# matsengrp/linearham

Measured on AMD Instinct MI355X. Metric: phylo-HMM log-likelihood evals/sec (100-leaf x 400-site family), higher is better.
Workload: dtype f64

## Files before the change

### linearham_amd/csrc/lh_capi.hip

```cpp
#include <algorithm>
#include <array>
#include <map>
#include <cstdio>
#include <cstring>
#include <functional>
#include <atomic>
#include <chrono>
#include <string>
#include <thread>
#include <utility>
#include <vector>

#include "lh_device.h"

namespace lh {
const DebugOptions& debug_options() {
  static const DebugOptions opts = [] {
    DebugOptions o;
    auto set = [](const char* name) { return std::getenv(name) != nullptr; };
    auto num = [](const char* name, int dflt) { const char* e = std::getenv(name); return e ? std::atoi(e) : dflt; };
    o.chunk = std::max(256, num("LH_CHUNK", o.chunk));
    o.host_sub = std::max(256, num("LH_HOST_SUB", o.host_sub));
    o.eval_split = std::min(8, std::max(0, num("LH_EVAL_SPLIT", o.eval_split)));
    o.eval_fwd_priority = std::min(1, num("LH_EVAL_FWD_PRIORITY", o.eval_fwd_priority));
    o.k2b_no_pair = set("LH_K2B_NO_PAIR");
    o.k2b_vd_single = set("LH_K2B_VD_SINGLE");
    o.sample_timing = set("LH_SAMPLE_TIMING");
    o.k1_tile_cap = num("LH_K1_TILE_CAP", 0);
    o.k1_cxx_walk = set("LH_K1_CXX_WALK");
    o.k1_tables = set("LH_K1_TABLES");
    o.k1_stack = set("LH_K1_STACK");
    o.k1_no_tables = set("LH_K1_NO_TABLES");
    o.k1_segments = set("LH_K1_SEGMENTS");
    o.k1_seg_waves = num("LH_K1_SEG_WAVES", o.k1_seg_waves);
    o.k1_no_fuse = set("LH_K1_NO_FUSE");
    o.codon_blocks = std::max(1, num("LH_CODON_BLOCKS", o.codon_blocks));
    o.events_blocks = std::max(1, num("LH_EVENTS_BLOCKS", o.events_blocks));
    o.anc_out_mb = std::max(1, num("LH_ANC_OUT_MB", o.anc_out_mb));
    o.edge_out_mb = std::max(1, num("LH_EDGE_OUT_MB", o.edge_out_mb));
    o.collect_hash_bits = std::min(64, std::max(1, num("LH_COLLECT_HASH_BITS", o.collect_hash_bits)));
    return o;
  }();
  return opts;
}
}

namespace {

thread_local std::string g_error;

int fail(const std::string& msg) {
  g_error = msg;
  return 1;
}

#define LH_HIP(expr)                                                                      \
  do {                                                                                    \
    hipError_t e_ = (expr);                                                               \
    if (e_ != hipSuccess)                                                                 \
      return fail(std::string(#expr) + ": " + hipGetErrorString(e_));                     \
  } while (0)

template <bool Pinned>
class Buffer {
 public:
  Buffer() = default;
  Buffer(const Buffer&) = delete;
  Buffer& operator=(const Buffer&) = delete;
  ~Buffer() { release(); }
  int ensure(size_t bytes) {
    bytes = std::max<size_t>(bytes, 64);
    if (bytes <= cap_) return 0;
    if (p_) {
      LH_HIP(hipDeviceSynchronize());
      release();
    }
// ... 199 lines not shown
struct SeqStore {
  DevBuf ids, flag, pairs;
  DevBuf gather_slots, gather_out;
  DevBuf store[2];
  int cur = 0;
  int32_t K = 0;
  size_t cap = 0;
};

struct CollectWs {
  DevBuf seqs, hash, states;
  int32_t n_last = -1;
  SeqStore store;
};

struct LineageWs {
  DevBuf naive, path, nt_hash, aa_hash;
  lh::LineageBatch last{};
  SeqStore store;
  LineageWs() { last.n = -1; }
};

struct HostInputs {
  DevBuf ops, brlen, er, pi, alpha;
  DevBuf rates, naive;
  DevBuf words;
  DevBuf log_offset;
  DevBuf em;
};
struct HostOutputs {
  DevBuf loglik, rates, xmsa_emission, forward, scaler_counts;
  DevBuf states;
  DevBuf anc, rate_choice;
  DevBuf weighted_sum, weight_stats;
  DevBuf log_cand, log_prior;
  DevBuf log_path;
};

struct HostPipe {
  PinnedBuf pinned[2];
  hipStream_t copy = nullptr, comp = nullptr;
  hipEvent_t staged[2] = {nullptr, nullptr};
  ~HostPipe() {
    for (hipEvent_t e : staged)
      if (e) (void)hipEventDestroy(e);
    if (copy) (void)hipStreamDestroy(copy);
    if (comp) (void)hipStreamDestroy(comp);
  }
};

struct OverlapPipe {
  static constexpr int kMaxSplit = 8;
  hipStream_t prune = nullptr, fwd = nullptr;
  hipEvent_t fork = nullptr, join_prune = nullptr, join_fwd = nullptr;
  hipEvent_t pruned[kMaxSplit] = {};
  bool ready = false;
  int ensure(bool fwd_high) {
    if (ready) return 0;
    int least = 0, greatest = 0;
    LH_HIP(hipDeviceGetStreamPriorityRange(&least, &greatest));
    if (!prune) LH_HIP(hipStreamCreateWithFlags(&prune, hipStreamNonBlocking));
    if (!fwd) LH_HIP(hipStreamCreateWithPriority(&fwd, hipStreamNonBlocking, fwd_high ? greatest : 0));
    for (hipEvent_t* e : {&fork, &join_prune, &join_fwd})
      if (!*e) LH_HIP(hipEventCreateWithFlags(e, hipEventDisableTiming));
    for (hipEvent_t& e : pruned)
      if (!e) LH_HIP(hipEventCreateWithFlags(&e, hipEventDisableTiming));
    ready = true;
    return 0;
  }
  ~OverlapPipe() {
    for (hipEvent_t e : {fork, join_prune, join_fwd})
      if (e) (void)hipEventDestroy(e);
    for (hipEvent_t e : pruned)
      if (e) (void)hipEventDestroy(e);
    if (prune) (void)hipStreamDestroy(prune);
    if (fwd) (void)hipStreamDestroy(fwd);
  }
};

}

struct lh_family {
  int device = 0;
  lh::DevFamily host{};
  lh::DevFamily* dev = nullptr;
  std::vector<void*> allocs;
  char* arena_ptr = nullptr;
  size_t arena_left = 0;
  Workspace ws;
  ForwardWs fws;
  AsrWs asr;
  PosteriorWs post;
  CandidateWs cand;
  ViterbiWs vit;
  CodonSource codon_src;
  CodonWs codon;
  EventsWs events;
  CollectWs collect;
  LineageWs lineage;
  AncestralWs anc;
  EdgesWs edges;
  DevBuf forward_dev;
  HostInputs in;
  HostOutputs out;
  PinnedBuf staging;
  HostPipe pipe;
  OverlapPipe overlap;
  bool profile = false;
  KernelTimer<3> eval_timer;
  KernelTimer<1> asr_timer, post_timer;
  KernelTimer<1> prior_timer, cand_timer;
  KernelTimer<1> collect_timer;
  KernelTimer<1> vit_timer;
  KernelTimer<1> codon_timer;
  KernelTimer<2> events_timer;
  KernelTimer<1> lineage_timer;
  KernelTimer<3> anc_timer;
  KernelTimer<3> edges_timer;
  KernelTimer<5> chain_timer;
  bool extended = false;
  bool have_sampler = false;
  lh::DevSampler sampler{};
  const lh::DevSampler* sampler_dev = nullptr;
  int32_t n_ucol_used = 0;
// ... 303 lines not shown

struct TreeBatch {
  int32_t n, T, max_depth;
  const int32_t* ops;
  const double* brlen;
  const double* er;
  const double* pi;
  const double* model;
  int32_t R;
  bool per_rate = false;
  size_t nodes() const { return 2 * (size_t)T - 2; }
  size_t n_ops() const { return (size_t)T - 2; }
  size_t model_stride() const { return per_rate ? (size_t)R : 1; }
  bool has_arrays() const { return ops && brlen && er && pi && model; }
  const int32_t* schedule(size_t i) const { return ops + i * n_ops() * 4; }
  TreeBatch slice(size_t off, int32_t m) const {
    return {m, T, max_depth, schedule(off), brlen + off * nodes(), er + off * 6, pi + off * 4, model + off * model_stride(),
            R, per_rate};
  }
  std::array<size_t, 5> sample_bytes() const {
    return {sizeof(int32_t) * 4 * n_ops(), sizeof(double) * nodes(), sizeof(double) * 6, sizeof(double) * 4,
            sizeof(double) * model_stride()};
  }
};

int check_batch(const lh_family* f, const std::string& w, const TreeBatch& b, bool needs_sampler = false) {
  const int n = b.n, T = b.T, R = b.R, max_depth = b.max_depth;
  if (!f) return fail(w + ": null family");
  if (needs_sampler && !f->have_sampler) return fail(w + ": lh_family_set_sampler has not been called");
  if (n < 0) return fail(w + ": negative batch size");
  if (n == 0) return -1;
  if (f->host.n_seqs < 1) return fail(w + ": family was created without an MSA (forward-only)");
  if (T != f->host.n_seqs + 1) return fail(w + ": n_tips must equal n_seqs + 1 (naive)");
  if (T < 3) return fail(w + ": need at least 3 tips");
  if (R < 1 || R > 64) return fail(w + ": num_rates out of range");
  if (max_depth < 0 || max_depth > 16) return fail(w + ": max_depth out of range");
  if ((size_t)T * 128 > 160 * 1024) return fail(w + ": too many tips for the LDS tip table");
  return 0;
}

size_t eval_bytes_per_sample(const lh_family* f, int T, int R) {
  return k1_bytes_per_sample(f, T, R) + sizeof(double) * R * 6 * (size_t)std::max(f->host.n_prune, 1);
}

size_t eval_group(const lh_family* f, int T, int R) {
  return std::min<size_t>(kChunk, std::max<size_t>(1024, ((size_t)16 << 30) / eval_bytes_per_sample(f, T, R)));
}

size_t asr_group(const lh_family* f, int T, int R, size_t clv_per_sample) {
  return std::min<size_t>(8192, std::max<size_t>(64, ((size_t)8 << 30) / (clv_per_sample + eval_bytes_per_sample(f, T, R))));
}

int prune_group(lh_family* f, const std::string& who, const TreeBatch& g, const double* rates, bool mix, hipStream_t stream,
                int* planes, size_t row0 = 0, int row0_planes = 0) {
  Workspace& w = f->ws;
  const lh::PruneWsSizes z = lh::prune_ws_sizes(g.T, f->host.msa_mixed_n != 0);
  const size_t L = (size_t)std::max(f->host.n_prune, 0), pl = (size_t)row0_planes;
  lh::PruneWs p = w.prune;
  p.scratch += row0 * g.R * z.scratch_doubles_per_rate;
  p.wops += row0 * g.n_ops();
  p.wlen += row0 * g.n_ops();
  p.tabs += row0 * z.tabs_per_sample;
  p.hdr += row0;
  *planes = lh::launch_prune(f->host, g.n, g.R, g.T, g.max_depth, g.ops, g.brlen, rates, w.eig.get<double>() + row0 * 36, p, g.pi,
                             w.site_lik.get<double>() + row0 * pl * 5 * L, w.site_scal.get<int32_t>() + row0 * pl * L, stream,
                             mix, f->extended || !mix);
  if (*planes < 0) return fail(who + ": " + lh::prune_last_error());
  f->k1_form = lh::prune_last_form();
  if (!mix && *planes != g.R && f->host.n_prune > 0) return fail(who + ": internal error (rate planes were mixed)");
  if (row0 > 0 && *planes != row0_planes) return fail(who + ": internal error (sub-batches with different rate planes)");
  return 0;
}

bool valid_op(const int32_t* op, int T, int nodes, int max_depth) {
  const int kind = op[0] & 15;
  const bool push = op[0] & lh::OP_PUSH_FLAG;
  const int rank = op[0] >> lh::OP_RANK_SHIFT;
  bool ok = (op[0] & 0xe0) == 0 && op[0] >= 0 && kind <= 2 && rank <= T - 3;
  if (kind == lh::OP_CHERRY) ok = ok && op[1] >= 1 && op[1] < T && op[2] >= 1 && op[2] < T;
  if (kind == lh::OP_TIP_ACC) ok = ok && !push && op[1] >= 1 && op[1] < T && op[2] >= T && op[2] < nodes;
  if (kind == lh::OP_POP_ACC) ok = ok && !push && op[1] >= T && op[1] < nodes && op[2] >= T && op[2] < nodes;
  if (push || kind == lh::OP_POP_ACC) ok = ok && op[3] >= 0 && op[3] < max_depth;
  return ok;
}

bool valid_schedule(const int32_t* ops, int T, int nodes, int max_depth) {
  int count = 0, depth = 0;
  for (int k = 0; k < T - 2; ++k) {
    const int32_t* op = ops + (size_t)k * 4;
    if (!valid_op(op, T, nodes, max_depth)) return false;
    const int kind = op[0] & 15, rank = op[0] >> lh::OP_RANK_SHIFT;
    if (kind == lh::OP_CHERRY) {
      if (rank != 0 && rank != count) return false;
      if (((op[0] & lh::OP_PUSH_FLAG) != 0) != (k != 0)) return false;
      if (k != 0 && op[3] != depth++) return false;
    } else {
      if (rank != count) return false;
      count += kind == lh::OP_POP_ACC ? 2 : 1;
      if (kind == lh::OP_POP_ACC && op[3] != --depth) return false;
    }
  }
  return count == T - 3 && depth == 0;
}

template <typename Fn>
void in_threads(size_t n, int nw, Fn&& fn) {
  if (nw <= 1) return fn((size_t)0, n);
  std::vector<std::thread> pool;
  for (int t = 0; t < nw; ++t) pool.emplace_back(fn, n * t / nw, n * (t + 1) / nw);
  for (std::thread& th : pool) th.join();
}

bool valid_schedules(const TreeBatch& b) {
  const size_t n = b.n;
  const int nw = (int)std::max<size_t>(1, std::min<size_t>({(size_t)std::thread::hardware_concurrency(), (size_t)8, n * b.n_ops() / 65536}));
  std::atomic<bool> bad{false};
  in_threads(n, nw, [&](size_t lo, size_t hi) {
    for (size_t i = lo; i < hi && !bad; ++i)
      if (!valid_schedule(b.schedule(i), b.T, (int)b.nodes(), b.max_depth)) bad = true;
// ... 618 lines not shown
      return fail("lh_family_set_sampler: D-J junction dimensions differ from the family's");
    if (upload_sampler_junction(f, desc->dj, &s.dj)) return 1;
    draws += (s.n_d >= 2) + s.dj.n_rows;
    s.states_per_sample += 1 + s.dj.n_rows;
  }
  s.words_per_sample = 2 * draws;
  f->sampler = s;
  if (upload(f, &s, 1, &f->sampler_dev)) return 1;
  f->have_sampler = true;
  return 0;
}

int32_t lh_sample_words(const lh_family* f) { return f && f->have_sampler ? f->sampler.words_per_sample : 0; }
int32_t lh_sample_states(const lh_family* f) { return f && f->have_sampler ? f->sampler.states_per_sample : 0; }

int lh_family_status(lh_family* f) {
  if (!f) return fail("lh_family_status: null family");
  DeviceGuard guard(f);
  return check_async_error(f, "lh_family_status");
}

int lh_profile_enable(lh_family* f, int enable) {
  if (!f) return fail("null family");
  f->profile = enable != 0;
  return 0;
}

int lh_profile_read(lh_family* f, double* ms_model, double* ms_prune, double* ms_forward, int64_t* n_launches) {
  double ms[3];
  if (profile_read(f, &lh_family::eval_timer, ms, n_launches)) return 1;
  if (ms_model) *ms_model = ms[0];
  if (ms_prune) *ms_prune = ms[1];
  if (ms_forward) *ms_forward = ms[2];
  return 0;
}

int lh_asr_profile_read(lh_family* f, double* ms_sampling, int64_t* n_launches) {
  return profile_read(f, &lh_family::asr_timer, ms_sampling, n_launches);
}

namespace {

constexpr int kEvalSplit = 1;
constexpr bool kEvalFwdHigh = false;
static_assert(kEvalSplit >= 1 && kEvalSplit <= OverlapPipe::kMaxSplit, "one `pruned` event per sub-batch");
int eval_sub_batch(int m) {
  const int forced = lh::debug_options().eval_split;
  if (forced > 0) return (m + forced - 1) / forced;
  constexpr int kBlock = 6144;
  if (kEvalSplit <= 1 || m < 2 * kBlock) return m;
  return ((m + kEvalSplit - 1) / kEvalSplit + kBlock - 1) / kBlock * kBlock;
}

int eval_group_split(lh_family* f, const TreeBatch& g, int off, int per, double* rates, double* em_out, double* loglik,
                     const lh_eval_outputs* outs, const lh::LogEmRequest& lem, hipStream_t stream) {
  OverlapPipe& op = f->overlap;
  const int fwd_priority = lh::debug_options().eval_fwd_priority;
  if (op.ensure(fwd_priority < 0 ? kEvalFwdHigh : fwd_priority > 0)) return 1;
  Workspace& w = f->ws;
  const int m = g.n, R = g.R;
  const size_t C = f->host.n_xmsa, L = (size_t)std::max(f->host.n_prune, 0);
  KernelTimer<3>* timer = f->profile ? &f->eval_timer : nullptr;
  LH_HIP(hipEventRecord(op.fork, stream));
  LH_HIP(hipStreamWaitEvent(op.prune, op.fork, 0));
  LH_HIP(hipStreamWaitEvent(op.fwd, op.fork, 0));
  auto enqueue = [&]() -> int {
    if (timer) timer->begin_spans();
    if (timer && timer->span_begin(0, op.prune)) return 1;
    lh::launch_model_setup(m, R, g.er, g.pi, g.model, rates, w.eig.get<double>(), op.prune);
    if (timer && timer->span_end(op.prune)) return 1;
    int planes = 0;
    for (int r0 = 0, j = 0; r0 < m; r0 += per, ++j) {
      const int k = std::min(per, m - r0);
      const TreeBatch sub = g.slice(r0, k);
      if (timer && timer->span_begin(1, op.prune)) return 1;
      if (prune_group(f, "lh_eval_batch", sub, rates + (size_t)r0 * R, true, op.prune, &planes, r0, planes)) return 1;
      if (timer && timer->span_end(op.prune)) return 1;
      LH_HIP(hipEventRecord(op.pruned[j], op.prune));
      LH_HIP(hipStreamWaitEvent(op.fwd, op.pruned[j], 0));
      if (timer && timer->span_begin(2, op.fwd)) return 1;
      const size_t s0 = (size_t)off + r0;
      const lh::LogEmRequest lem_k{lem.cols, lem.n, lem.out ? lem.out + s0 * lem.n : nullptr};
      if (run_forward(f, k, planes, w.site_lik.get<double>() + (size_t)r0 * planes * 5 * L,
                      w.site_scal.get<int32_t>() + (size_t)r0 * planes * L, sub.pi, nullptr,
                      em_out ? em_out + (size_t)r0 * C : nullptr, loglik + s0, outs, s0, op.fwd, lem_k, r0, m))
        return 1;
      if (timer && timer->span_end(op.fwd)) return 1;
    }
    if (timer) timer->end_spans();
    return 0;
  };
  const int rc = enqueue();
  LH_HIP(hipEventRecord(op.join_prune, op.prune));
  LH_HIP(hipEventRecord(op.join_fwd, op.fwd));
  LH_HIP(hipStreamWaitEvent(stream, op.join_prune, 0));
  LH_HIP(hipStreamWaitEvent(stream, op.join_fwd, 0));
  return rc;
}

int eval_device(lh_family* f, const TreeBatch& b, double* loglik, const lh_eval_outputs* outs, void* hip_stream,
                const lh::LogEmRequest& lem = lh::LogEmRequest{}, const std::function<int(int, int)>* after = nullptr) {
  if (int rc = check_batch(f, "lh_eval_batch", b)) return rc > 0;
  DeviceGuard guard(f);
  if (!b.has_arrays() || !loglik) return fail("lh_eval_batch: null array");
  hipStream_t stream = static_cast<hipStream_t>(hip_stream);
  const int n = b.n, R = b.R;
  const int chunk = (int)std::min<size_t>(n, eval_group(f, b.T, R));
  if (ensure_workspace(f, chunk, R, b.T)) return 1;
  Workspace& w = f->ws;
  double *eig = w.eig.get<double>(), *site_lik = w.site_lik.get<double>();
  int32_t* site_scal = w.site_scal.get<int32_t>();
  const size_t C = f->host.n_xmsa;
  for (int off = 0; off < n; off += chunk) {
    const int m = std::min(chunk, n - off);
    const TreeBatch g = b.slice(off, m);
    double* rates = (outs && outs->rates) ? outs->rates + (size_t)off * R : w.rates.get<double>();
    double* em_out = (outs && outs->xmsa_emission) ? outs->xmsa_emission + (size_t)off * C : nullptr;
    if (const int per = eval_sub_batch(m); per < m) {
      if (eval_group_split(f, g, off, per, rates, em_out, loglik, outs, lem, stream)) return 1;
      LH_HIP(hipGetLastError());
      if (after && (*after)(off, m)) return 1;
      continue;
    }
    if (f->profile && f->eval_timer.begin(stream)) return 1;
    lh::launch_model_setup(m, R, g.er, g.pi, g.model, rates, eig, stream);
    if (f->profile && f->eval_timer.mark(1, stream)) return 1;
    int planes = 0;
    if (prune_group(f, "lh_eval_batch", g, rates, true, stream, &planes)) return 1;
    if (f->profile && f->eval_timer.mark(2, stream)) return 1;
    const lh::LogEmRequest lem_m{lem.cols, lem.n, lem.out ? lem.out + (size_t)off * lem.n : nullptr};
    if (run_forward(f, m, planes, site_lik, site_scal, g.pi, nullptr, em_out, loglik + off, outs, off, stream, lem_m))
      return 1;
    if (f->profile && f->eval_timer.end(stream)) return 1;
    LH_HIP(hipGetLastError());
    if (after && (*after)(off, m)) return 1;
  }
  return 0;
}

}

int lh_eval_batch_device(lh_family* f, int32_t n, int32_t T, int32_t max_depth, const int32_t* ops,
                         const double* brlen, const double* er, const double* pi, const double* alpha,
                         int32_t R, double* loglik, const lh_eval_outputs* outs, void* hip_stream) {
  return eval_device(f, {n, T, max_depth, ops, brlen, er, pi, alpha, R}, loglik, outs, hip_stream);
}

int lh_eval_batch(lh_family* f, int32_t n, int32_t T, int32_t max_depth, const int32_t* ops,
                  const double* brlen, const double* er, const double* pi, const double* alpha, int32_t R,
                  double* loglik, const lh_eval_outputs* outs) {
  const TreeBatch host{n, T, max_depth, ops, brlen, er, pi, alpha, R};
  if (int rc = check_batch(f, "lh_eval_batch", host)) return rc > 0;
  DeviceGuard guard(f);
  if (!host.has_arrays() || !loglik) return fail("lh_eval_batch: null array");
  const size_t C = f->host.n_xmsa, FS = f->host.forward_size, SS = f->host.scaler_size;
  const lh_eval_outputs none{};
  const lh_eval_outputs& o = outs ? *outs : none;
  HostOutputs& out = f->out;
  lh_eval_outputs d_outs{};
  if (out.loglik.ensure(sizeof(double) * n) || out_buf(o.rates, out.rates, sizeof(double) * R * n, &d_outs.rates) ||
      out_buf(o.xmsa_emission, out.xmsa_emission, sizeof(double) * C * n, &d_outs.xmsa_emission) ||
      out_buf(o.forward, out.forward, sizeof(double) * FS * n, &d_outs.forward) ||
      out_buf(o.scaler_counts, out.scaler_counts, sizeof(int32_t) * SS * n, &d_outs.scaler_counts))
    return 1;
  double* d_ll = out.loglik.get<double>();

  const std::array<size_t, 5> bytes = host.sample_bytes();
  const char* src[5] = {(const char*)ops, (const char*)brlen, (const char*)er, (const char*)pi, (const char*)alpha};
  DevBuf* in[5] = {&f->in.ops, &f->in.brlen, &f->in.er, &f->in.pi, &f->in.alpha};
  char* dst[5];
  size_t per_sample = 0;
  for (int a = 0; a < 5; ++a) {
    if (in[a]->ensure(bytes[a] * n)) return 1;
    dst[a] = in[a]->get<char>();
    per_sample += bytes[a];
  }
  const TreeBatch dev{n, T, max_depth, (const int32_t*)dst[0], (const double*)dst[1], (const double*)dst[2],
                      (const double*)dst[3], (const double*)dst[4], R};
  const int kSub = lh::debug_options().host_sub;
  const int sub = std::min<int>(n, kSub);
  HostPipe& hp = f->pipe;
// ... 2059 lines not shown
```

### linearham_amd/csrc/lh_device.h

```cpp
#pragma once
#include <hip/hip_runtime.h>
#include <stdint.h>

#include "linearham_amd.h"

namespace lh {

constexpr double kScaleFactor = 0x1p256;
constexpr double kScaleThreshold = 0x1p-256;
constexpr double kLogScaleFactor = 177.445678223345993274;

enum : int { OP_CHERRY = 0, OP_TIP_ACC = 1, OP_POP_ACC = 2, OP_PUSH_FLAG = 16, OP_RANK_SHIFT = 8 };

enum : int { W_CHERRY = 0, W_TIP_ACC = 1, W_POP = 2, W_CTIP = 3, W_CTAB_ACC = 4 };

struct PruneWs {
  double* scratch;
  int2* wops;
  double* wlen;
  int4* tabs;
  int4* hdr;
  int32_t* err_flag;
};
struct PruneWsSizes {
  size_t scratch_doubles_per_rate;
  size_t tabs_per_sample;
};
PruneWsSizes prune_ws_sizes(int T, bool mixed_n);

struct DevSegments {
  int32_t n_genes;
  int32_t n_chunks;
  int32_t cons_sites;
  int32_t cons_diffs;
  const uint16_t* cons_col;
  const uint32_t* cons_rng;
  const uint32_t* cons_dif;
  const uint4* inds_c;
};

struct DevJunction {
  int32_t n_rows, n_left, n_right;
  int32_t left_pad, right_pad;
  const double *enter_lo;
  const double *left_trans;
  const double *left_lo;
  const int32_t* left_xmsa;
  const double *right_gp_nli;
  const double *right_ntt;
  const double *right_nlo;
  const double *right_trans, *right_gp_li;
  const int32_t *right_xmsa;
  const int32_t *nti_xmsa;
  const double *exit_nlo;
  const double *exit_trans, *exit_gp_li;
  const int32_t* row_pat;
};

struct DevFamily {
  int32_t has_d, n_seqs, n_sites, n_xmsa;
  int32_t n_pat;
  int32_t n_prune;
  int32_t msa_mixed_n;
  int32_t n_ucol;
  int32_t idx_byte_offsets;
  const uint8_t* msa;
  const uint64_t* msa_planes;
  const int32_t* site_pat;
  const int32_t* u_pat;
  const uint8_t* u_base;
  const int32_t* ucol_of_col;
  const int32_t* col_of_ucol;
  DevSegments vpadding, vgerm, dgerm, jgerm, jpadding;
  const double *vgerm_gene_prob, *vpadding_transition, *vgerm_trans_prod, *jpadding_transition;
  DevJunction vd, dj;
  int32_t max_genes;
  int32_t n_jcols;
  const int32_t* jcols;
  int64_t gem_size;
  int64_t forward_size;
  int64_t scaler_size;
// ... 121 lines not shown

struct LineageBatch {
  int32_t n, T, L, P;
  const uint8_t* anc;
  const uint8_t* naive;
  const int32_t* path;
  uint64_t hash_mask;
  int32_t draws = 1;
};
__host__ __device__ inline size_t n_slots(const LineageBatch& b) {
  return b.n > 0 ? (size_t)b.n * (size_t)b.draws * (b.P + 1) : 0;
}
__device__ inline const uint8_t* slot_row(const LineageBatch& b, int v, int s) {
  const int i = b.draws > 1 ? v / b.draws : v;
  if (s == b.P) return b.naive + (size_t)i * b.L;
  const int node = b.path[(size_t)i * b.P + s];
  if (node < b.T || node >= 2 * b.T - 2) return nullptr;
  return b.anc + ((size_t)v * (b.T - 2) + (node - b.T)) * b.L;
}
__device__ inline const uint8_t* slot_row(const LineageBatch& b, int x) { return slot_row(b, x / (b.P + 1), x % (b.P + 1)); }
constexpr uint64_t kLineagePadHash = 0;
void launch_lineage(const LineageBatch& b, uint64_t* nt_hash, uint64_t* aa_hash, hipStream_t stream);

template <class Rows>
void launch_store_verify(const Rows& src, int K, const int32_t* ids, const uint8_t* store, uint8_t* flag,
                         hipStream_t stream);
template <class Rows>
void launch_store_append(const Rows& src, int K, int n_pairs, const int32_t* pairs, uint8_t* store, hipStream_t stream);
template <class Rows>
void launch_store_gather(const Rows& src, int n_out, const int32_t* slots, uint8_t* out, hipStream_t stream);

__device__ static inline void compute_pmatrix(const double* __restrict__ e, double tr, double P[4][4]) {
  double ex[4];
#pragma unroll
  for (int k = 1; k < 4; ++k) ex[k] = expm1(e[k] * tr);
#pragma unroll
  for (int i = 0; i < 4; ++i)
#pragma unroll
    for (int j = 0; j < 4; ++j) {
      double v = (i == j) ? 1.0 : 0.0;
#pragma unroll
      for (int k = 1; k < 4; ++k) v = fma(e[4 + i * 4 + k] * ex[k], e[20 + k * 4 + j], v);
      P[i][j] = fmax(v, 0.0);
    }
}


void launch_model_setup(int n, int R, const double* er, const double* pi, const double* alpha,
                        double* rates, double* eig, hipStream_t stream);

int launch_prune(const DevFamily& fam, int n, int R, int T, int max_depth, const int32_t* ops,
                 const double* brlen, const double* rates, const double* eig, const PruneWs& ws, const double* pi,
                 double* site_lik, int32_t* site_scal, hipStream_t stream, bool allow_fused = true,
                 bool test_every_op = false);
const char* prune_last_form();
const char* prune_last_error();

void launch_gtr_setup(int n, const double* er, const double* pi, double* eig, hipStream_t stream);

int launch_asr(const DevFamily& fam, int n, int R, int T, const int32_t* ops, const double* brlen, const double* rates,
               const double* eig, const double* pi, const double* site_lik, const int32_t* site_scal,
               const uint8_t* naive, uint64_t seed, uint64_t sample0, double* clv, void* desc, uint8_t* anc,
               uint8_t* rate_choice, const int4* hdr , hipStream_t stream,
               int draws = 1);
size_t asr_desc_bytes(int T);
size_t asr_lds_bytes(int T, int L, int R, int n_prune);
size_t asr_slots(int L, int R);

struct AsrOp {
  int4 a, b;
};

void launch_asr_sched(int n, int T, const int32_t* ops, const int4* hdr, void* desc, hipStream_t stream);

struct AncWs {
  double* clv;
  double* part;
  double* tvec;
  double* rho;
  int32_t* chain;
  int32_t* plen;
  void* desc;
};
struct AncWsBytes {
  size_t clv, part, tvec, rho, chain;
  size_t total() const { return clv + part + tvec + rho + chain; }
};
AncWsBytes anc_ws_bytes(int T, int L, int R, int n_prune, int P);
size_t anc_lds_bytes(int T);
int launch_ancestral(const DevFamily& fam, int n, int R, int T, const int32_t* ops, const double* brlen, const double* rates,
                     const double* eig, const double* pi, const double* site_lik, const int32_t* site_scal,
                     const double* naive_prob, const int32_t* path, int P, const AncWs& ws, double* marg, double* rate_post,
                     const int4* hdr, int32_t* err_flag, hipStream_t stream);
void launch_site_base(int n, int L, size_t forward_size, const int32_t* off, const int32_t* idx, const double* post,
                      const double* loglik, double* site_base, hipStream_t stream);
void launch_ancestral_ends(int n, int P, int L, const int32_t* plen, const double* marg, const double* loglik, double* ends,
                           double* ll_used, hipStream_t stream);
void launch_ancestral_front(const DevFamily& fam, int n, int R, int T, const int32_t* ops, const double* pi,
                            const double* site_lik, const int32_t* site_scal, const double* naive_prob, const int32_t* path,
                            int P, const AncWs& ws, double* rate_post, const int4* hdr, int32_t* err_flag, hipStream_t stream);
size_t anc_lp(int n_prune);

__device__ static __forceinline__ void anc_tip_col(const double* tiptab, int tip, int st, double (&c)[4]) {
  const double* t = tiptab + tip * 16;
  if (st < 4) {
#pragma unroll
    for (int i = 0; i < 4; ++i) c[i] = t[st * 4 + i];
// ... 75 lines not shown
      double2* ck = clv_s + (size_t)k * 2 * plane + pat;
      ck[0] = make_double2(a[0], a[1]);
      ck[plane] = make_double2(a[2], a[3]);
    }
  }
}

struct SubWs {
  double* cc;
  double* ne;
  double* se;
  double* el;
  double* edge;
};
struct SubWsBytes {
  size_t cc, ne, se, el, edge;
  size_t total(bool with_edge) const { return cc + ne + se + el + (with_edge ? edge : 0); }
};
SubWsBytes sub_ws_bytes(int L, int R, int P);
size_t sub_lds_bytes(int T, int P);
struct SubOut {
  double *edge, *naive_edge, *chain_counts, *seed_edge, *edge_load, *rate_post;
};
int launch_substitutions(const DevFamily& fam, int n, int R, int T, const int32_t* ops, const double* brlen, const double* rates,
                         const double* eig, const double* pi, const double* site_lik, const int32_t* site_scal,
                         const double* naive_prob, const int32_t* path, int P, int seed_tip, const AncWs& ws, const SubWs& sws,
                         const SubOut& out, const int4* hdr, int32_t* err_flag, hipStream_t stream);

struct LogEmRequest {
  const int32_t* cols = nullptr;
  int n = 0;
  double* out = nullptr;
};
void launch_forward(const DevFamily& fam, const DevFamily* fam_dev, int n, int R, const double* site_lik,
                    const int32_t* site_scal, const double* pi, const double* em_in, double* em_out, double* gem,
                    int32_t* gcnt, double* jem,
                    int32_t* jrs, double* dxf, int32_t* dxc, double* loglik, double* forward_out, int32_t* scaler_out,
                    bool extended, hipStream_t stream, const LogEmRequest& lem = LogEmRequest{});
size_t forward_lds_bytes(const DevFamily& fam);
const char* forward_last_form();

size_t viterbi_bp_bytes(const DevFamily& fam);
size_t viterbi_lds_bytes(const DevFamily& fam);
void launch_viterbi(const DevFamily& fam, const DevSampler* smp_dev, int n, const double* gem, const int32_t* gcnt,
                    const double* jem, const int32_t* jrs, const double* loglik, uint8_t* bp, int32_t* states,
                    double* log_path, bool extended, hipStream_t stream);
void launch_path_prior(const DevFamily& fam, const DevSampler* smp_dev, int K, const int32_t* states, double* log_prior,
                       int32_t* first_bad, hipStream_t stream);

struct DebugOptions {
  int chunk = 49152;
  int host_sub = 12288;
  int eval_split = 0;
  int eval_fwd_priority = -1;
  bool k2b_no_pair = false;
  bool k2b_vd_single = false;
  bool sample_timing = false;
  int k1_tile_cap = 0;
  bool k1_cxx_walk = false;
  bool k1_tables = false;
  bool k1_stack = false;
  bool k1_no_tables = false;
  bool k1_segments = false;
  int k1_seg_waves = 4;
  bool k1_no_fuse = false;
  int codon_blocks = 2048;
  int events_blocks = 1024;
  int anc_out_mb = 4096;
  int edge_out_mb = 4096;
  int collect_hash_bits = 64;
};
const DebugOptions& debug_options();

}
```

### linearham_amd/csrc/lh_forward.hip

```cpp
#include <cstdio>
#include <cstdlib>

#include "lh_device.h"

namespace lh {

constexpr int kFwdThreads = 256;
constexpr int kFwdWaves = kFwdThreads / 64;
constexpr int kJunctionWaves = 4;

thread_local char g_k2a_form[64] = "", g_k2b_form[32] = "", g_forward_form[160] = "";

__device__ static inline int block_max_int(int v, int* red, int phase) {
#pragma unroll
  for (int off = 32; off > 0; off >>= 1) v = max(v, __shfl_xor(v, off, 64));
  int* r = red + phase * kFwdWaves;
  if ((threadIdx.x & 63) == 0) r[threadIdx.x >> 6] = v;
  __syncthreads();
  return max(max(r[0], r[1]), max(r[2], r[3]));
}

__device__ static inline int block_min_int(int v, int* red, int phase) {
  return -block_max_int(-v, red, phase);
}
// ... 160 lines not shown
#pragma unroll
  for (int q = 0; q < kG; ++q)
    if (tid + kFwdThreads * q < n && v[q] > 0.0) local_min = min(local_min, c[q]);
  int mn = block_min_int(local_min, redi, phase);
  if (mn == 0x3fffffff) mn = 0;
#pragma unroll
  for (int q = 0; q < kG; ++q) {
    const int g = tid + kFwdThreads * q;
    if (g < n) {
      double x = v[q];
      for (int d = c[q] - mn; d > 0 && x != 0.0; --d) x *= kScaleThreshold;
      out[g] = x;
    }
  }
  return mn;
}

__host__ __device__ static inline int cons_capacity(const DevFamily& fam) {
  int m = fam.vpadding.cons_sites;
  m = m > fam.vgerm.cons_sites ? m : fam.vgerm.cons_sites;
  m = m > fam.dgerm.cons_sites ? m : fam.dgerm.cons_sites;
  m = m > fam.jgerm.cons_sites ? m : fam.jgerm.cons_sites;
  m = m > fam.jpadding.cons_sites ? m : fam.jpadding.cons_sites;
  return m > 0 ? (m + 3) & ~1 : 0;
}

__host__ __device__ static inline bool small_sets_by_wave(const DevFamily& fam, bool ext, bool direct) {
  return !ext && fam.dgerm.n_genes <= 64 && fam.jgerm.n_genes <= 64 &&
         (direct || (fam.dgerm.cons_sites == 0 && fam.jgerm.cons_sites == 0 && fam.jpadding.cons_sites == 0));
}

struct ScaledProd {
  double v;
  int k;
};
__device__ static inline ScaledProd sp_mul(ScaledProd a, ScaledProd b) {
  ScaledProd r{a.v * b.v, a.k + b.k};
  if (r.v < kScaleThreshold) {
    r.v *= kScaleFactor;
    ++r.k;
  }
  return r;
}

__device__ static inline ScaledProd sp_from(double e) {
  ScaledProd r{e, 0};
  while (r.v < kScaleThreshold) {
    r.v *= kScaleFactor;
    ++r.k;
  }
  return r;
}

template <int kG, bool kByteOff>
__device__ static int fill_consensus(const DevSegments& seg, const double* em, int tid, double* __restrict__ out,
                                     int* redi, int phase, double* cons_inv, double* cons_pv, int* cons_pk,
                                     int cap) {
  const int ns = seg.cons_sites, n = seg.n_genes;
  auto em_at = [&](unsigned x) {
    return kByteOff ? *reinterpret_cast<const double*>(reinterpret_cast<const char*>(em) + x) : em[x];
  };
  ScaledProd x0{1.0, 0}, x1{1.0, 0};
  const int j0 = 2 * tid;
  if (j0 < ns) {
    const double e = em_at(seg.cons_col[j0]);
    cons_inv[j0] = fast_rcp(e);
    x0 = sp_from(e);
  }
  if (j0 + 1 < ns) {
    const double e = em_at(seg.cons_col[j0 + 1]);
    cons_inv[j0 + 1] = fast_rcp(e);
    x1 = sp_from(e);
  }
  if (tid == 0) cons_inv[ns] = 1.0;
  ScaledProd incl = sp_mul(x0, x1);
  const int lane = tid & 63, wave = tid >> 6;
#pragma unroll
  for (int off = 1; off < 64; off <<= 1) {
    const double ov = __shfl_up(incl.v, off, 64);
    const int ok = __shfl_up(incl.k, off, 64);
    if (lane >= off) incl = sp_mul(ScaledProd{ov, ok}, incl);
  }
  if (lane == 63) {
    cons_pv[cap + wave] = incl.v;
    cons_pk[cap + wave] = incl.k;
  }
  __syncthreads();
  ScaledProd excl = incl;
  {
    const double ov = __shfl_up(incl.v, 1, 64);
    const int ok = __shfl_up(incl.k, 1, 64);
    excl = lane == 0 ? ScaledProd{1.0, 0} : ScaledProd{ov, ok};
    for (int w = 0; w < wave; ++w) excl = sp_mul(ScaledProd{cons_pv[cap + w], cons_pk[cap + w]}, excl);
  }
  if (j0 <= ns) {
    cons_pv[j0] = excl.v;
    cons_pk[j0] = excl.k;
  }
  if (j0 + 1 <= ns) {
    const ScaledProd p1 = sp_mul(excl, x0);
    cons_pv[j0 + 1] = p1.v;
    cons_pk[j0 + 1] = p1.k;
  }
  __syncthreads();

  double v[kG];
  int c[kG];
#pragma unroll
  for (int q = 0; q < kG; ++q) {
    v[q] = 1.0;
    c[q] = 0;
    const int g = tid + kFwdThreads * q;
    if (g < n) {
      const unsigned rng = seg.cons_rng[g];
      const int a = rng & 0xffffu, b = (rng >> 16) & 0x1ffu;
      double r = cons_pv[b] * fast_rcp(cons_pv[a]);
      int k = cons_pk[b] - cons_pk[a];
      const uint32_t* dp = seg.cons_dif + g;
      const int n_dif = 8 * (int)(rng >> 25);
      uint32_t w_next[8];
#pragma unroll
      for (int i = 0; i < 8; ++i) w_next[i] = n_dif > 0 ? dp[(size_t)i * n] : 0u;
      for (int d = 0; d < n_dif; d += 8) {
        uint32_t w[8];
#pragma unroll
        for (int i = 0; i < 8; ++i) w[i] = w_next[i];
        if (d + 8 < n_dif) {
#pragma unroll
          for (int i = 0; i < 8; ++i) w_next[i] = dp[(size_t)(d + 8 + i) * n];
        }
        double fct[8];
#pragma unroll
        for (int i = 0; i < 8; ++i) fct[i] = em_at(w[i] >> 16) * cons_inv[w[i] & 0xffffu];
#pragma unroll
        for (int i = 0; i < 8; ++i) {
          r *= fct[i];
          if (r < kScaleThreshold) {
            r *= kScaleFactor;
            ++k;
          } else if (r >= kScaleFactor) {
            r *= kScaleThreshold;
            --k;
          }
        }
      }
      while (r < kScaleThreshold) {
        r *= kScaleFactor;
        ++k;
      }
      while (k > 0 && r >= 1.0) {
        r *= kScaleThreshold;
        --k;
      }
      while (k < 0) {
        r *= kScaleFactor;
        ++k;
      }
      v[q] = r;
      c[q] = k;
    }
  }
  int local_max = 0;
#pragma unroll
  for (int q = 0; q < kG; ++q)
    if (tid + kFwdThreads * q < n) local_max = max(local_max, c[q]);
  const int mx = block_max_int(local_max, redi, phase);
#pragma unroll
  for (int q = 0; q < kG; ++q) {
    const int g = tid + kFwdThreads * q;
    if (g < n) out[g] = v[q] * pow_scale(mx - c[q]);
  }
  return mx;
}

template <int kG, bool kFromSiteLik, bool kByteOff, bool kExt = false, bool kLem = false>
__global__ void __launch_bounds__(kFwdThreads) __attribute__((amdgpu_num_sgpr(80)))
    emission_kernel(const DevFamily* __restrict__ fam_dev, int R, const double* __restrict__ site_lik,
                    const int32_t* __restrict__ site_scal, const double* __restrict__ pi,
                    const double* __restrict__ em_in, double* __restrict__ em_out, double* __restrict__ gem_all,
                    int32_t* __restrict__ gcnt_all, double* __restrict__ jem_all, int32_t* __restrict__ jrs_all,
                    const int32_t* __restrict__ lem_cols, int n_lem, double* __restrict__ lem_all) {
  const DevFamily& fam = *fam_dev;
  extern __shared__ double em[];
  const size_t s = blockIdx.x;
  const int tid = threadIdx.x;
  const int C = fam.n_ucol;
  double* inv_pi = em + ((C + 2) & ~1);
  int* redi = reinterpret_cast<int*>(inv_pi + 6);
  int* em_bad = redi + 2 * kFwdWaves;
  const int cons_cap = cons_capacity(fam);
  double* cons_inv = reinterpret_cast<double*>(redi + 2 * kFwdWaves + 2);
  double* cons_pv = cons_inv + cons_cap;
  int* cons_pk = reinterpret_cast<int*>(cons_pv + cons_cap + 4);
  int* ems = cons_pk + (cons_cap ? cons_cap + 4 : 0);
  if (tid == 0) *em_bad = 0;
// ... 1281 lines not shown
```

### linearham_amd/csrc/lh_prune.hip

```cpp
#include <cstdlib>

#include <cstdio>
#include <type_traits>

#include "lh_device.h"

namespace lh {

namespace {

thread_local char g_prune_form[64] = "";
thread_local char g_prune_error[256] = "";

#define LH_SLOT_COPY(dst, src)                       \
  _Pragma("unroll") for (int s_ = 0; s_ < S; ++s_) { \
    dst[s_][0] = src[s_][0];                         \
    dst[s_][1] = src[s_][1];                         \
    dst[s_][2] = src[s_][2];                         \
    dst[s_][3] = src[s_][3];                         \
  }
#define LH_PUSH_IF(d)                                   \
  if constexpr (kDepth > d) {                           \
    if (push_mask & (1u << d)) { LH_SLOT_COPY(st##d, a) } \
  }
// ... 1225 lines not shown
  }
}

#define LH_PRUNE_CT_KERNEL(NAME, WAVES)                                                              \
  template <int kDepth, bool kN, bool kFused, bool kAsm>                                             \
  __global__ void __launch_bounds__(1024) __attribute__((amdgpu_waves_per_eu(WAVES, WAVES))) NAME(   \
      const PruneCtArgs args ) {                                         \
    prune_body_ct<kDepth, kN, kFused, kAsm>();                                                       \
  }
LH_PRUNE_CT_KERNEL(prune_kernel_ct6, 6)
LH_PRUNE_CT_KERNEL(prune_kernel_ct5, 5)
LH_PRUNE_CT_KERNEL(prune_kernel_ct4, 4)
#undef LH_PRUNE_CT_KERNEL
#define LH_PRUNE_PARAMS                                                                                     \
  int n_samples, int n2, int tile, int R, int wpr, const uint8_t *__restrict__ msa, int L, int T, int n_ops, \
      const int32_t *__restrict__ ops, const int4 *__restrict__ hdr, int32_t *err_flag,                     \
      const double *__restrict__ brlen, const double *__restrict__ rates, const double *__restrict__ eig,  \
      double *pmat_w, size_t rate_stride, const double *__restrict__ pi,                                   \
      double *__restrict__ site_lik, int32_t *__restrict__ site_scal
#define LH_PRUNE_ARGS \
  n2, tile, R, wpr, msa, L, T, n_ops, ops, hdr, err_flag, brlen, rates, eig, pmat_w, rate_stride, pi, site_lik, site_scal
#define LH_PRUNE_SAMPLES(BODY) BODY((int)blockIdx.z, LH_PRUNE_ARGS);

#define LH_PRUNE_KERNEL(NAME, WAVES)                                                                 \
  template <int kDepth, bool kN>                                                                     \
  __global__ void __launch_bounds__(1024) __attribute__((amdgpu_waves_per_eu(WAVES, WAVES))) NAME(   \
      LH_PRUNE_PARAMS) {                                                                             \
    LH_PRUNE_SAMPLES((prune_body<kDepth, true, kN, true>))                                           \
  }
LH_PRUNE_KERNEL(prune_kernel_w6, 6)
LH_PRUNE_KERNEL(prune_kernel_w5, 5)
LH_PRUNE_KERNEL(prune_kernel_w4, 4)
#undef LH_PRUNE_KERNEL

template <int kDepth, bool kN>
__global__ void __launch_bounds__(512) __attribute__((amdgpu_waves_per_eu(5, 5))) prune_kernel_seg(LH_PRUNE_PARAMS) {
  LH_PRUNE_SAMPLES((prune_body<kDepth, true, kN, false, true>))
}
template <int kDepth, bool kN>
__global__ void __launch_bounds__(512) __attribute__((amdgpu_waves_per_eu(4, 4))) prune_kernel_seg4(LH_PRUNE_PARAMS) {
  LH_PRUNE_SAMPLES((prune_body<kDepth, true, kN, false, true>))
}

PruneWsSizes prune_ws_sizes(int T, bool mixed_n) {
  PruneWsSizes z;
  z.tabs_per_sample = (size_t)std::max((T - 1) / 2, 1);
  const size_t e = mixed_n ? 25 : 16;
  z.scratch_doubles_per_rate = std::max((size_t)std::max(T - 3, 0) * 16 + z.tabs_per_sample * e * 4, (size_t)std::max(T - 2, 1) * 32);
  return z;
}

int launch_prune(const DevFamily& fam, int n, int R, int T, int max_depth, const int32_t* ops,
                 const double* brlen, const double* rates, const double* eig, const PruneWs& ws, const double* pi,
                 double* site_lik, int32_t* site_scal, hipStream_t stream, bool allow_fused, bool test_every_op) {
  const int L = fam.n_prune;
  const PruneWsSizes sizes = prune_ws_sizes(T, fam.msa_mixed_n != 0);
  if (L == 0) {
    hipLaunchKernelGGL(schedule_stack_check_kernel, dim3(n), dim3(64), 0, stream, T, std::max(max_depth, 1), 0, ops, ws.hdr, ws.err_flag);
    return R;
  }
  double* pmat = ws.scratch;
  const size_t rate_stride = sizes.scratch_doubles_per_rate;
  const DebugOptions& dbg = debug_options();
  const int cap_env = dbg.k1_tile_cap;
  const int cap = cap_env >= 64 ? std::min(cap_env, 1024) : 1024;
  const int tiles = (L + cap - 1) / cap;
  const int tile = tiles == 1 ? L : (((L + tiles - 1) / tiles + 127) & ~127);
  int n2 = tile / 128, n1;
  {
    const int rem = tile - 128 * n2;
    if (rem > 64) {
      ++n2;
      n1 = 0;
    } else {
      n1 = rem > 0 ? 1 : 0;
    }
  }
  const int wpr = n2 + n1;
  const size_t tip_bytes = (size_t)T * 16 * sizeof(double);
  const size_t pad = (size_t)n2 * 128 + (size_t)n1 * 64;
  const size_t tail_bytes = (((size_t)std::max(T - 2, 1) * sizeof(int2)) + 31) & ~(size_t)15;
  const bool mixed = fam.msa_mixed_n != 0;
  const size_t ones_bytes = mixed ? 32 : 0;
  const size_t fused_lds = std::max((size_t)R * tip_bytes + ones_bytes + tail_bytes, (size_t)R * pad * (5 * sizeof(double) + sizeof(int)));
  const bool fused = allow_fused && !dbg.k1_no_fuse && !dbg.k1_segments &&
                     ((R * wpr <= 8 && fused_lds <= 53 * 1024) ||
                      (R * wpr > 8 && R * wpr <= kCtFusedMaxWaves && fused_lds <= kCtFusedMaxLds));
  const bool big = !fused && ((160 * 1024 / tip_bytes) * wpr / 4 < 5 || dbg.k1_segments);
  const bool tables_hook = dbg.k1_tables || dbg.k1_no_tables;
  const bool use_asm = !dbg.k1_cxx_walk && !test_every_op;
  const bool stack_fused = fused && max_depth <= 4 && dbg.k1_stack && !tables_hook;
  const bool seg = big && max_depth <= 4 && !tables_hook;
  const size_t seg_bytes = (size_t)(2 * kSegOps + 1) * 16 * sizeof(double) + ones_bytes;
  size_t lds = fused ? fused_lds : seg ? seg_bytes : tip_bytes + ones_bytes + tail_bytes;
  if (lds > 160 * 1024) {
    snprintf(g_prune_error, sizeof(g_prune_error),
             "K1: a tree of %d tips with stack depth %d needs %zu bytes of LDS in the cherry-table form (160 KB per CU)", T, max_depth, lds);
    return -1;
  }
  if (stack_fused || seg) {
    hipLaunchKernelGGL(schedule_stack_check_kernel, dim3(n), dim3(64), 0, stream, T, stack_fused && max_depth <= 3 ? 3 : 4,
                       stack_fused ? 1 : 0, ops, ws.hdr, ws.err_flag);
  } else {
    hipLaunchKernelGGL(schedule_rewrite_kernel, dim3(n), dim3(64), (sizes.tabs_per_sample + 16) * sizeof(int), stream, T, max_depth,
                       (int)sizes.tabs_per_sample, dbg.k1_no_tables ? 0 : 1, ops, brlen, ws.wops, ws.wlen, ws.tabs, ws.hdr, ws.err_flag);
  }
  const int wg_waves = fused ? R * wpr : wpr;
  dim3 grid(tiles, fused ? 1 : R, n), block(64 * wg_waves);
  const int n_ops = T - 2;
  hipError_t attr_rc = hipSuccess;
#define LH_LAUNCH_K(K, NAME)                                                                                     \
  {                                                                                                              \
    if (lds > 64 * 1024)                                                                                         \
      attr_rc = hipFuncSetAttribute(reinterpret_cast<const void*>(K), hipFuncAttributeMaxDynamicSharedMemorySize, (int)lds); \
    snprintf(g_prune_form, sizeof(g_prune_form), "%s", NAME);                                                    \
    if (attr_rc == hipSuccess)                                                                                   \
      hipLaunchKernelGGL(K, grid, block, lds, stream, n, n2, tile, R, wpr, fam.msa, L, T, n_ops, ops, ws.hdr, ws.err_flag, \
                         brlen, rates, eig, pmat, rate_stride, pi, site_lik, site_scal);                        \
  }
#define LH_LAUNCH_CT(K, NAME)                                                                                    \
  {                                                                                                              \
    if (lds > 64 * 1024)                                                                                         \
      attr_rc = hipFuncSetAttribute(reinterpret_cast<const void*>(K), hipFuncAttributeMaxDynamicSharedMemorySize, (int)lds); \
    snprintf(g_prune_form, sizeof(g_prune_form), "%s", NAME);                                                    \
    if (attr_rc == hipSuccess) hipLaunchKernelGGL(K, grid, block, lds, stream, ct_args);                        \
  }
  PruneCtArgs ct_args = {};
  ct_args.n2 = n2, ct_args.tile = tile, ct_args.R = R, ct_args.wpr = wpr;
  ct_args.L = L, ct_args.T = T, ct_args.tabs_stride = (int)sizes.tabs_per_sample;
  ct_args.msa = fam.msa, ct_args.planes = fam.msa_planes;
  ct_args.wops = ws.wops, ct_args.wlen = ws.wlen, ct_args.tabs = ws.tabs, ct_args.hdr = ws.hdr;
  ct_args.brlen = brlen, ct_args.rates = rates, ct_args.eig = eig;
  ct_args.pmat_w = pmat, ct_args.rate_stride = rate_stride;
  ct_args.pi = pi, ct_args.site_lik = site_lik, ct_args.site_scal = site_scal;
  const int lds_waves = lds == 0 ? 8 : (int)((160 * 1024 / lds) * wg_waves / 4);
  if (stack_fused) {
#define LH_LAUNCH_STACK(D, N)                                                          \
  {                                                                                    \
    if (lds_waves >= 6 && D == 3)                                                      \
      LH_LAUNCH_K((prune_kernel_w6<D, N>), "w6<" #D "," #N ">")                        \
    else if (lds_waves >= 5)                                                           \
      LH_LAUNCH_K((prune_kernel_w5<D, N>), "w5<" #D "," #N ">")                        \
    else                                                                               \
      LH_LAUNCH_K((prune_kernel_w4<D, N>), "w4<" #D "," #N ">")                        \
  }
    if (max_depth <= 3 && !mixed)
      LH_LAUNCH_STACK(3, false)
    else if (max_depth <= 3)
      LH_LAUNCH_STACK(3, true)
    else if (!mixed)
      LH_LAUNCH_STACK(4, false)
    else
      LH_LAUNCH_STACK(4, true)
#undef LH_LAUNCH_STACK
  } else if (seg) {
    if (dbg.k1_seg_waves == 4) {
      if (mixed)
        LH_LAUNCH_K((prune_kernel_seg4<4, true>), "seg4<4,true>")
      else
// ... 58 lines not shown
```

Before: 8.659 million.

## Overlap model setup with prune schedule kernel and batch consensus rescaling

Runs the model-setup kernel (K0) on a side stream so it overlaps the prune schedule-check/rewrite kernel, joining the streams before the main prune kernel through a new PruneFork callback. This applies to both the split-eval path and the plain eval path, and an env var keeps the old serial order. Separately, the forward consensus fill checks whether all eight factors and the running product sit in a safe exponent range. When every lane passes, it multiplies all eight and rescales once instead of after each factor. The changes add stream and event bookkeeping and a wave-wide ballot branch in exchange for less serialization and fewer per-step compares.

After: 8.747 million, median of 6. +1.0%, better.

```diff
diff --git a/linearham_amd/csrc/lh_capi.hip b/linearham_amd/csrc/lh_capi.hip
--- a/linearham_amd/csrc/lh_capi.hip
+++ b/linearham_amd/csrc/lh_capi.hip
@@ -22,6 +22,7 @@
     o.chunk = std::max(256, num("LH_CHUNK", o.chunk));
     o.host_sub = std::max(256, num("LH_HOST_SUB", o.host_sub));
     o.eval_split = std::min(8, std::max(0, num("LH_EVAL_SPLIT", o.eval_split)));
+    o.k0_serial = set("LH_K0_SERIAL");
     o.eval_fwd_priority = std::min(1, num("LH_EVAL_FWD_PRIORITY", o.eval_fwd_priority));
     o.k2b_no_pair = set("LH_K2B_NO_PAIR");
     o.k2b_vd_single = set("LH_K2B_VD_SINGLE");
@@ -327,7 +328,7 @@
 struct OverlapPipe {
   static constexpr int kMaxSplit = 8;
   hipStream_t prune = nullptr, fwd = nullptr;
-  hipEvent_t fork = nullptr, join_prune = nullptr, join_fwd = nullptr;
+  hipEvent_t fork = nullptr, join_prune = nullptr, join_fwd = nullptr, k0a = nullptr;
   hipEvent_t pruned[kMaxSplit] = {};
   bool ready = false;
   int ensure(bool fwd_high) {
@@ -336,7 +337,7 @@
     LH_HIP(hipDeviceGetStreamPriorityRange(&least, &greatest));
     if (!prune) LH_HIP(hipStreamCreateWithFlags(&prune, hipStreamNonBlocking));
     if (!fwd) LH_HIP(hipStreamCreateWithPriority(&fwd, hipStreamNonBlocking, fwd_high ? greatest : 0));
-    for (hipEvent_t* e : {&fork, &join_prune, &join_fwd})
+    for (hipEvent_t* e : {&fork, &join_prune, &join_fwd, &k0a})
       if (!*e) LH_HIP(hipEventCreateWithFlags(e, hipEventDisableTiming));
     for (hipEvent_t& e : pruned)
       if (!e) LH_HIP(hipEventCreateWithFlags(&e, hipEventDisableTiming));
@@ -344,7 +345,7 @@
     return 0;
   }
   ~OverlapPipe() {
-    for (hipEvent_t e : {fork, join_prune, join_fwd})
+    for (hipEvent_t e : {fork, join_prune, join_fwd, k0a})
       if (e) (void)hipEventDestroy(e);
     for (hipEvent_t e : pruned)
       if (e) (void)hipEventDestroy(e);
@@ -754,7 +755,7 @@
 }
 
 int prune_group(lh_family* f, const std::string& who, const TreeBatch& g, const double* rates, bool mix, hipStream_t stream,
-                int* planes, size_t row0 = 0, int row0_planes = 0) {
+                int* planes, size_t row0 = 0, int row0_planes = 0, const lh::PruneFork* fork = nullptr) {
   Workspace& w = f->ws;
   const lh::PruneWsSizes z = lh::prune_ws_sizes(g.T, f->host.msa_mixed_n != 0);
   const size_t L = (size_t)std::max(f->host.n_prune, 0), pl = (size_t)row0_planes;
@@ -766,7 +767,7 @@
   p.hdr += row0;
   *planes = lh::launch_prune(f->host, g.n, g.R, g.T, g.max_depth, g.ops, g.brlen, rates, w.eig.get<double>() + row0 * 36, p, g.pi,
                              w.site_lik.get<double>() + row0 * pl * 5 * L, w.site_scal.get<int32_t>() + row0 * pl * L, stream,
-                             mix, f->extended || !mix);
+                             mix, f->extended || !mix, fork);
   if (*planes < 0) return fail(who + ": " + lh::prune_last_error());
   f->k1_form = lh::prune_last_form();
   if (!mix && *planes != g.R && f->host.n_prune > 0) return fail(who + ": internal error (rate planes were mixed)");
@@ -1491,11 +1492,15 @@
   return ((m + kEvalSplit - 1) / kEvalSplit + kBlock - 1) / kBlock * kBlock;
 }
 
+int ensure_overlap(lh_family* f) {
+  const int fwd_priority = lh::debug_options().eval_fwd_priority;
+  return f->overlap.ensure(fwd_priority < 0 ? kEvalFwdHigh : fwd_priority > 0);
+}
+
 int eval_group_split(lh_family* f, const TreeBatch& g, int off, int per, double* rates, double* em_out, double* loglik,
                      const lh_eval_outputs* outs, const lh::LogEmRequest& lem, hipStream_t stream) {
   OverlapPipe& op = f->overlap;
-  const int fwd_priority = lh::debug_options().eval_fwd_priority;
-  if (op.ensure(fwd_priority < 0 ? kEvalFwdHigh : fwd_priority > 0)) return 1;
+  if (ensure_overlap(f)) return 1;
   Workspace& w = f->ws;
   const int m = g.n, R = g.R;
   const size_t C = f->host.n_xmsa, L = (size_t)std::max(f->host.n_prune, 0);
@@ -1503,17 +1508,27 @@
   LH_HIP(hipEventRecord(op.fork, stream));
   LH_HIP(hipStreamWaitEvent(op.prune, op.fork, 0));
   LH_HIP(hipStreamWaitEvent(op.fwd, op.fork, 0));
+  const bool beside = !lh::debug_options().k0_serial;
+  hipStream_t k0a_stream = beside ? op.fwd : op.prune;
+  const lh::PruneFork k0_fork{op.prune, [&]() -> int {
+                                LH_HIP(hipStreamWaitEvent(op.prune, op.k0a, 0));
+                                if (timer && (timer->span_end(op.prune) || timer->span_begin(1, op.prune))) return 1;
+                                return 0;
+                              }};
   auto enqueue = [&]() -> int {
     if (timer) timer->begin_spans();
-    if (timer && timer->span_begin(0, op.prune)) return 1;
-    lh::launch_model_setup(m, R, g.er, g.pi, g.model, rates, w.eig.get<double>(), op.prune);
-    if (timer && timer->span_end(op.prune)) return 1;
+    if (timer && timer->span_begin(0, k0a_stream)) return 1;
+    lh::launch_model_setup(m, R, g.er, g.pi, g.model, rates, w.eig.get<double>(), k0a_stream);
+    if (beside) LH_HIP(hipEventRecord(op.k0a, op.fwd));
+    if (!beside && timer && timer->span_end(op.prune)) return 1;
     int planes = 0;
     for (int r0 = 0, j = 0; r0 < m; r0 += per, ++j) {
       const int k = std::min(per, m - r0);
       const TreeBatch sub = g.slice(r0, k);
-      if (timer && timer->span_begin(1, op.prune)) return 1;
-      if (prune_group(f, "lh_eval_batch", sub, rates + (size_t)r0 * R, true, op.prune, &planes, r0, planes)) return 1;
+      const bool forked = beside && r0 == 0;
+      if (!forked && timer && timer->span_begin(1, op.prune)) return 1;
+      if (prune_group(f, "lh_eval_batch", sub, rates + (size_t)r0 * R, true, op.prune, &planes, r0, planes, forked ? &k0_fork : nullptr))
+        return 1;
       if (timer && timer->span_end(op.prune)) return 1;
       LH_HIP(hipEventRecord(op.pruned[j], op.prune));
       LH_HIP(hipStreamWaitEvent(op.fwd, op.pruned[j], 0));
@@ -1550,6 +1565,8 @@
   double *eig = w.eig.get<double>(), *site_lik = w.site_lik.get<double>();
   int32_t* site_scal = w.site_scal.get<int32_t>();
   const size_t C = f->host.n_xmsa;
+  const bool serial_k0 = lh::debug_options().k0_serial;
+  if (!serial_k0 && ensure_overlap(f)) return 1;
   for (int off = 0; off < n; off += chunk) {
     const int m = std::min(chunk, n - off);
     const TreeBatch g = b.slice(off, m);
@@ -1562,10 +1579,27 @@
       continue;
     }
     if (f->profile && f->eval_timer.begin(stream)) return 1;
-    lh::launch_model_setup(m, R, g.er, g.pi, g.model, rates, eig, stream);
-    if (f->profile && f->eval_timer.mark(1, stream)) return 1;
     int planes = 0;
-    if (prune_group(f, "lh_eval_batch", g, rates, true, stream, &planes)) return 1;
+    if (serial_k0) {
+      lh::launch_model_setup(m, R, g.er, g.pi, g.model, rates, eig, stream);
+      if (f->profile && f->eval_timer.mark(1, stream)) return 1;
+      if (prune_group(f, "lh_eval_batch", g, rates, true, stream, &planes)) return 1;
+    } else {
+      OverlapPipe& op = f->overlap;
+      LH_HIP(hipEventRecord(op.fork, stream));
+      LH_HIP(hipStreamWaitEvent(op.prune, op.fork, 0));
+      lh::launch_model_setup(m, R, g.er, g.pi, g.model, rates, eig, op.prune);
+      LH_HIP(hipEventRecord(op.join_prune, op.prune));
+      bool joined = false;
+      const lh::PruneFork k0_fork{stream, [&]() -> int {
+                                    joined = true;
+                                    LH_HIP(hipStreamWaitEvent(stream, op.join_prune, 0));
+                                    return f->profile ? f->eval_timer.mark(1, stream) : 0;
+                                  }};
+      const int rc = prune_group(f, "lh_eval_batch", g, rates, true, stream, &planes, 0, 0, &k0_fork);
+      if (!joined) LH_HIP(hipStreamWaitEvent(stream, op.join_prune, 0));
+      if (rc) return 1;
+    }
     if (f->profile && f->eval_timer.mark(2, stream)) return 1;
     const lh::LogEmRequest lem_m{lem.cols, lem.n, lem.out ? lem.out + (size_t)off * lem.n : nullptr};
     if (run_forward(f, m, planes, site_lik, site_scal, g.pi, nullptr, em_out, loglik + off, outs, off, stream, lem_m))
diff --git a/linearham_amd/csrc/lh_device.h b/linearham_amd/csrc/lh_device.h
--- a/linearham_amd/csrc/lh_device.h
+++ b/linearham_amd/csrc/lh_device.h
@@ -1,6 +1,8 @@
 #pragma once
 #include <hip/hip_runtime.h>
 #include <stdint.h>
+
+#include <functional>
 
 #include "linearham_amd.h"
 
@@ -27,6 +29,10 @@
   size_t tabs_per_sample;
 };
 PruneWsSizes prune_ws_sizes(int T, bool mixed_n);
+struct PruneFork {
+  hipStream_t sched;
+  std::function<int()> join;
+};
 
 struct DevSegments {
   int32_t n_genes;
@@ -254,7 +260,7 @@
 int launch_prune(const DevFamily& fam, int n, int R, int T, int max_depth, const int32_t* ops,
                  const double* brlen, const double* rates, const double* eig, const PruneWs& ws, const double* pi,
                  double* site_lik, int32_t* site_scal, hipStream_t stream, bool allow_fused = true,
-                 bool test_every_op = false);
+                 bool test_every_op = false, const PruneFork* fork = nullptr);
 const char* prune_last_form();
 const char* prune_last_error();
 
@@ -436,6 +442,7 @@
   int chunk = 49152;
   int host_sub = 12288;
   int eval_split = 0;
+  bool k0_serial = false;
   int eval_fwd_priority = -1;
   bool k2b_no_pair = false;
   bool k2b_vd_single = false;
diff --git a/linearham_amd/csrc/lh_forward.hip b/linearham_amd/csrc/lh_forward.hip
--- a/linearham_amd/csrc/lh_forward.hip
+++ b/linearham_amd/csrc/lh_forward.hip
@@ -236,8 +236,11 @@
   return r;
 }
 
+constexpr uint32_t kHi2m256 = (1023u - 256u) << 20, kHi2m64 = (1023u - 64u) << 20;
+constexpr uint32_t kHi2p64 = (1023u + 64u) << 20, kHi2p256 = (1023u + 256u) << 20;
+
 template <int kG, bool kByteOff>
-__device__ static int fill_consensus(const DevSegments& seg, const double* em, int tid, double* __restrict__ out,
+__device__ static __forceinline__ int fill_consensus(const DevSegments& seg, const double* em, int tid, double* __restrict__ out,
                                      int* redi, int phase, double* cons_inv, double* cons_pv, int* cons_pk,
                                      int cap) {
   const int ns = seg.cons_sites, n = seg.n_genes;
@@ -316,15 +319,36 @@
         double fct[8];
 #pragma unroll
         for (int i = 0; i < 8; ++i) fct[i] = em_at(w[i] >> 16) * cons_inv[w[i] & 0xffffu];
-#pragma unroll
-        for (int i = 0; i < 8; ++i) {
-          r *= fct[i];
-          if (r < kScaleThreshold) {
+        uint32_t lo = (uint32_t)__double2hiint(fct[0]), hi = lo;
+#pragma unroll
+        for (int i = 1; i < 8; ++i) {
+          const uint32_t h = (uint32_t)__double2hiint(fct[i]);
+          lo = min(lo, h);
+          hi = max(hi, h);
+        }
+        const bool safe = lo >= kHi2m64 && hi < kHi2p64 && (uint32_t)__double2hiint(r) - kHi2m256 < kHi2p256 - kHi2m256;
+        if (__ballot(!safe) == 0) {
+#pragma unroll
+          for (int i = 0; i < 8; ++i) r *= fct[i];
+          while (r < kScaleThreshold) {
             r *= kScaleFactor;
             ++k;
-          } else if (r >= kScaleFactor) {
+          }
+          while (r >= kScaleFactor) {
             r *= kScaleThreshold;
             --k;
+          }
+        } else {
+#pragma unroll
+          for (int i = 0; i < 8; ++i) {
+            r *= fct[i];
+            if (r < kScaleThreshold) {
+              r *= kScaleFactor;
+              ++k;
+            } else if (r >= kScaleFactor) {
+              r *= kScaleThreshold;
+              --k;
+            }
           }
         }
       }
diff --git a/linearham_amd/csrc/lh_prune.hip b/linearham_amd/csrc/lh_prune.hip
--- a/linearham_amd/csrc/lh_prune.hip
+++ b/linearham_amd/csrc/lh_prune.hip
@@ -1301,12 +1301,19 @@
 
 int launch_prune(const DevFamily& fam, int n, int R, int T, int max_depth, const int32_t* ops,
                  const double* brlen, const double* rates, const double* eig, const PruneWs& ws, const double* pi,
-                 double* site_lik, int32_t* site_scal, hipStream_t stream, bool allow_fused, bool test_every_op) {
+                 double* site_lik, int32_t* site_scal, hipStream_t stream, bool allow_fused, bool test_every_op,
+                 const PruneFork* fork) {
+  hipStream_t sched = fork ? fork->sched : stream;
+  auto joined = [&]() {
+    if (!fork || fork->join() == 0) return true;
+    snprintf(g_prune_error, sizeof(g_prune_error), "K1: the schedule kernel's stream could not be joined");
+    return false;
+  };
   const int L = fam.n_prune;
   const PruneWsSizes sizes = prune_ws_sizes(T, fam.msa_mixed_n != 0);
   if (L == 0) {
-    hipLaunchKernelGGL(schedule_stack_check_kernel, dim3(n), dim3(64), 0, stream, T, std::max(max_depth, 1), 0, ops, ws.hdr, ws.err_flag);
-    return R;
+    hipLaunchKernelGGL(schedule_stack_check_kernel, dim3(n), dim3(64), 0, sched, T, std::max(max_depth, 1), 0, ops, ws.hdr, ws.err_flag);
+    return joined() ? R : -1;
   }
   double* pmat = ws.scratch;
   const size_t rate_stride = sizes.scratch_doubles_per_rate;
@@ -1348,12 +1355,13 @@
     return -1;
   }
   if (stack_fused || seg) {
-    hipLaunchKernelGGL(schedule_stack_check_kernel, dim3(n), dim3(64), 0, stream, T, stack_fused && max_depth <= 3 ? 3 : 4,
+    hipLaunchKernelGGL(schedule_stack_check_kernel, dim3(n), dim3(64), 0, sched, T, stack_fused && max_depth <= 3 ? 3 : 4,
                        stack_fused ? 1 : 0, ops, ws.hdr, ws.err_flag);
   } else {
-    hipLaunchKernelGGL(schedule_rewrite_kernel, dim3(n), dim3(64), (sizes.tabs_per_sample + 16) * sizeof(int), stream, T, max_depth,
+    hipLaunchKernelGGL(schedule_rewrite_kernel, dim3(n), dim3(64), (sizes.tabs_per_sample + 16) * sizeof(int), sched, T, max_depth,
                        (int)sizes.tabs_per_sample, dbg.k1_no_tables ? 0 : 1, ops, brlen, ws.wops, ws.wlen, ws.tabs, ws.hdr, ws.err_flag);
   }
+  if (!joined()) return -1;
   const int wg_waves = fused ? R * wpr : wpr;
   dim3 grid(tiles, fused ? 1 : R, n), block(64 * wg_waves);
   const int n_ops = T - 2;
```
